# RupertLuo/Valley

Measured on AMD Instinct MI355X. Metric: frames/sec ViT-L/14 encode + prefill tokens/sec (13B), higher is better.
Workload: dtype bf16

## Files before the change

valley_amd/csrc/attention.hip:

```cpp
#include <cstdlib>
#include "common.hpp"
#include "../../include/valley_hip.h"

namespace {

constexpr float LOG2E = 1.4426950408889634f;
constexpr float NEG_BIG = -1.0e30f;

#ifndef VLY_DECODE_MERGE_FENCE
#define VLY_DECODE_MERGE_FENCE 0
#endif
#ifndef VLY_VIT_PRIO
#define VLY_VIT_PRIO 0
#endif
#ifndef VLY_VIT_STAGGER
#define VLY_VIT_STAGGER 0
#endif
#ifndef VLY_VIT_TIMING
#define VLY_VIT_TIMING 0
#endif
#ifndef VLY_VIT_STAGE2
#define VLY_VIT_STAGE2 1
#endif
#ifndef VLY_VIT_ROT
#define VLY_VIT_ROT 0
#endif
#ifndef VLY_VIT_FOLD
#define VLY_VIT_FOLD 0
#endif
#ifndef VLY_VIT_STORE_LINES
#define VLY_VIT_STORE_LINES 0
#endif
#ifndef VLY_FAST_EXP2
#define VLY_FAST_EXP2 1
#endif
VLY_DEVICE float sm_exp2(float x) {
#if VLY_FAST_EXP2
    return __builtin_amdgcn_exp2f(x);
#else
    return exp2f(x);
#endif
}

VLY_DEVICE uint32_t sel16(const u32x4& a, const u32x4& b, int dd) {
    const uint32_t w = dd < 8 ? a[dd >> 1] : b[(dd - 8) >> 1];
    return (dd & 1) ? (w >> 16) : (w & 0xffffu);
}

VLY_DEVICE int opaque_i32(int v) {
    asm volatile("" : "+v"(v));
    return v;
}

VLY_DEVICE void store_tile_rows(uint16_t* row_ptr, const f32x4 (&o)[4], float inv, int g) {
    uint32_t y[2][4];
#pragma unroll
    for (int w = 0; w < 2; ++w) {
        uint32_t d[4];
#pragma unroll
        for (int dt = 0; dt < 4; ++dt) d[dt] = pack_h2(o[dt][2 * w] * inv, o[dt][2 * w + 1] * inv);
        const auto p01 = __builtin_amdgcn_permlane16_swap(d[0], d[1], false, false);
        const auto p23 = __builtin_amdgcn_permlane16_swap(d[2], d[3], false, false);
        const auto q0 = __builtin_amdgcn_permlane32_swap(p01[0], p23[0], false, false);
        const auto q1 = __builtin_amdgcn_permlane32_swap(p01[1], p23[1], false, false);
        y[w][0] = q0[0]; y[w][1] = q1[0]; y[w][2] = q0[1]; y[w][3] = q1[1];
    }
    u32x4* dst = (u32x4*)(row_ptr + 16 * g);
    dst[0] = u32x4{y[0][0], y[1][0], y[0][1], y[1][1]};
    dst[1] = u32x4{y[0][2], y[1][2], y[0][3], y[1][3]};
}

template <typename OP>
VLY_DEVICE float rows4_reduce(float v, OP op) {
    {
        const uint32_t x = __float_as_uint(v);
        const auto r = __builtin_amdgcn_permlane16_swap(x, x, false, false);
        v = op(__uint_as_float(r[0]), __uint_as_float(r[1]));
    }
    {
        const uint32_t x = __float_as_uint(v);
        const auto r = __builtin_amdgcn_permlane32_swap(x, x, false, false);
        v = op(__uint_as_float(r[0]), __uint_as_float(r[1]));
    }
    return v;
}
VLY_DEVICE float rows4_max(float v) { return rows4_reduce(v, [](float a, float b) { return fmaxf(a, b); }); }
VLY_DEVICE float rows4_sum(float v) { return rows4_reduce(v, [](float a, float b) { return a + b; }); }

constexpr int VN = 257;
constexpr int VNT = 17;
constexpr int VNC = 9;
constexpr int VLD = 3072;
constexpr int VT_STRIDE = 296;
constexpr int VK_BYTES = VNT * 16 * 128;

constexpr int VNW = 8;

#if VLY_VIT_TIMING
constexpr int VTS_WG = 4096, VTS_N = 24;
__device__ unsigned long long vit_ts[VTS_WG * VNW * VTS_N];
#define VLY_VSTAMP()                                                                                     \
    do {                                                                                                  \
        if (ts_row && lane == 0 && tsn < VTS_N) ts_row[tsn] = __builtin_readcyclecounter();                \
        ++tsn;                                                                                            \
    } while (0)
#else
#define VLY_VSTAMP() do {} while (0)
#endif

__global__ void __launch_bounds__(VNW * 64, 4) vit_attn_kernel(const uint16_t* __restrict__ qkv, uint16_t* __restrict__ out) {
    __shared__ __attribute__((aligned(16))) char smem[VK_BYTES + 64 * VT_STRIDE * 2];
    char* sK = smem;
    uint16_t* sVt = (uint16_t*)(smem + VK_BYTES);

    const int tid = threadIdx.x, lane = tid & 63, wave = tid >> 6;
    const int l15 = lane & 15, g = lane >> 4;
    [[maybe_unused]] const int hi16 = opaque_i32(16);
    const int h = blockIdx.x & 15;
#if VLY_VIT_TIMING
    int tsn = 0;
    unsigned long long* ts_row = blockIdx.x < VTS_WG ? vit_ts + ((size_t)blockIdx.x * VNW + wave) * VTS_N : nullptr;
    VLY_VSTAMP();
    if (ts_row && lane == 0) {
        unsigned hw, xcc;
        asm volatile("s_getreg_b32 %0, hwreg(HW_REG_HW_ID)" : "=s"(hw));
        asm volatile("s_getreg_b32 %0, hwreg(HW_REG_XCC_ID)" : "=s"(xcc));
        ts_row[tsn] = (unsigned long long)hw | ((unsigned long long)xcc << 32);
    }
    ++tsn;
#endif
    const int f = blockIdx.x >> 4;
    const uint16_t* base = qkv + (size_t)f * VN * VLD + h * 64;

#if VLY_VIT_STAGE2
    const int dq = wave & 3;
    u32x4 kr[5];
#pragma unroll
    for (int i = 0; i < 5; ++i) {
        const int sl = tid + i * VNW * 64, row = min(sl >> 3, VN - 1), c = sl & 7;
        kr[i] = *(const u32x4*)(base + (size_t)row * VLD + 1024 + c * 8);
    }
    u32x4 vr[2][4];
#pragma unroll
    for (int ps = 0; ps < 2; ++ps) {
        const int pg = ps == 0 ? (wave >> 2) : 2, kv0 = 2 * (pg * 64 + lane), kv1 = kv0 + 1;
        if (ps == 0 || wave < 4) {
            const uint16_t* r0 = base + (size_t)min(kv0, VN - 1) * VLD + 2048 + dq * 16;
            const uint16_t* r1 = base + (size_t)min(kv1, VN - 1) * VLD + 2048 + dq * 16;
            vr[ps][0] = *(const u32x4*)r0;
            vr[ps][1] = *(const u32x4*)(r0 + 8);
            vr[ps][2] = *(const u32x4*)r1;
            vr[ps][3] = *(const u32x4*)(r1 + 8);
        }
// ... 234 lines not shown
#if VLY_VIT_TIMING
    if (ts_row && lane == 0 && tsn < VTS_N) ts_row[VTS_N - 1] = (unsigned long long)tsn;
#endif
}
#undef VLY_VSTAMP

typedef __attribute__((ext_vector_type(4))) short s16x4;
#include "attention_vit_persist.inc"
#include "attention_vit_pp.inc"

#ifndef VLY_LNW
#define VLY_LNW 8
#endif
constexpr int LNW = VLY_LNW;

VLY_DEVICE bf16x8 vt_frag256(const char* lo_addr) {
    typedef __attribute__((address_space(3))) s16x4 lds_s16x4;
    const s16x4 lo = __builtin_amdgcn_ds_read_tr16_b64_v4i16((lds_s16x4*)(lo_addr));
    const s16x4 hi = __builtin_amdgcn_ds_read_tr16_b64_v4i16((lds_s16x4*)(lo_addr + 16 * 256));
    return bf16x8{lo[0], lo[1], lo[2], lo[3], hi[0], hi[1], hi[2], hi[3]};
}

constexpr int L2_TILE = 64 * 256;
constexpr int L2_BUF = 2 * L2_TILE;

__global__ void __launch_bounds__(LNW * 64, 4) llama_attn2_kernel(const uint16_t* __restrict__ qkv, const uint16_t* __restrict__ kc,
                                                                 const uint16_t* __restrict__ vc, const uint8_t* __restrict__ key_valid,
                                                                 uint16_t* __restrict__ out, int S, int heads, int past,
                                                                 const int32_t* __restrict__ past_dev, int kv_stride, int ctx_max) {
    static_assert(LNW == 8, "16 + 16 pieces on 8 waves");
    __shared__ __attribute__((aligned(16))) char smem[2 * L2_BUF];
    const int tid = threadIdx.x, lane = tid & 63;
    const int wave = __builtin_amdgcn_readfirstlane(tid >> 6);
    const int l15 = lane & 15, g = lane >> 4;
    const int h = blockIdx.x, b = blockIdx.y, qb = (int)gridDim.z - 1 - (int)blockIdx.z;
    const int Hq = heads * 128;
    if (past_dev) past = min(*past_dev, ctx_max - S);
    const int kv_len = past + S;

    const int q = qb * (LNW * 16) + wave * 16 + l15;
    const int qc = min(q, S - 1);
    const int qpos = past + q;
    const int q_last = min(qb * (LNW * 16) + LNW * 16 - 1, S - 1);
    const int wave_qpos_max = past + min(qb * (LNW * 16) + wave * 16 + 15, S - 1);
    const int kv_end = min(past + q_last + 1, kv_len);
    const int ntiles = (kv_end + 63) >> 6;

    const size_t head_off = ((size_t)b * heads + h) * (size_t)ctx_max * 128;
    const __amdgpu_buffer_rsrc_t rsK = vly_rsrc(kc + head_off), rsV = vly_rsrc(vc + head_off);
    const __amdgpu_buffer_rsrc_t rsM = vly_rsrc(key_valid ? key_valid + (size_t)b * kv_stride : key_valid);
    const uint32_t lds0 = (uint32_t)(uintptr_t)(__attribute__((address_space(3))) char*)smem;
    const uint32_t hb = 0u;
    uint32_t okraw = 1u;
    bool okin = false;
    auto stage = [&](int kt, int buf) {
        const int kv0 = kt * 64;
#pragma unroll
        for (int pp = 0; pp < 2; ++pp) {
            const int pc = 2 * wave + pp, row = 4 * pc + (lane >> 4), cp = lane & 15;
            const uint32_t rb = hb + (uint32_t)min(kv0 + row, kv_len - 1) * 256u;
            const uint32_t voK = rb + (uint32_t)((cp ^ (row & 15)) << 4);
            const uint32_t voV = rb + (uint32_t)((cp ^ ((row & 7) << 1)) << 4);
            const uint32_t dst = __builtin_amdgcn_readfirstlane(lds0 + (uint32_t)buf * L2_BUF + (uint32_t)pc * 1024u);
            asm volatile("s_mov_b32 m0, %0" ::"s"(dst) : "memory");
            asm volatile("s_nop 0" ::: "memory");
            asm volatile("buffer_load_dwordx4 %0, %1, 0 offen lds" ::"v"(voK), "s"(rsK) : "memory");
            asm volatile("s_mov_b32 m0, %0" ::"s"(dst + (uint32_t)L2_TILE) : "memory");
            asm volatile("s_nop 0" ::: "memory");
            asm volatile("buffer_load_dwordx4 %0, %1, 0 offen lds" ::"v"(voV), "s"(rsV) : "memory");
        }
        const int kvl = kv0 + lane;
        okin = kvl < kv_len;
        if (key_valid) okraw = (uint32_t)__builtin_amdgcn_raw_buffer_load_b8(rsM, (uint32_t)min(kvl, kv_len - 1), 0, 0);
    };
    const int vr = 4 * g + (l15 >> 2);
    const int vbase0 = L2_TILE + vr * 256 + (l15 & 1) * 8 + (((l15 & 3) >> 1) << 4), vx0 = (vr & 7) << 5;

    if (ntiles > 0) stage(0, 0);
    const uint16_t* qp = qkv + ((size_t)b * S + qc) * 3 * Hq + h * 128;
    bf16x8 qf[4];
#pragma unroll
    for (int kk = 0; kk < 4; ++kk) qf[kk] = *(const bf16x8*)(qp + kk * 32 + g * 8);

    const float sc = 0.08838834764831845f * LOG2E;
    float m = NEG_BIG, l = 0.f;
    f32x4 o[8];
#pragma unroll
    for (int dt = 0; dt < 8; ++dt) o[dt] = f32x4{0.f, 0.f, 0.f, 0.f};

    for (int kt = 0; kt < ntiles; ++kt) {
        const int kv0 = kt * 64, buf = kt & 1;
        const char* sK = smem + buf * L2_BUF;
        __builtin_amdgcn_s_waitcnt(0x0f70);
        __syncthreads();
        const unsigned long long vmask = __ballot(okin && (okraw & 0xffu) != 0u);
        if (kt + 1 < ntiles) stage(kt + 1, buf ^ 1);
        if (kv0 > wave_qpos_max) continue;
        const int vbase = opaque_i32(vbase0), vx = opaque_i32(vx0);

        f32x4 s[4];
#pragma unroll
        for (int t = 0; t < 4; ++t) {
            f32x4 acc = {0.f, 0.f, 0.f, 0.f};
#pragma unroll
            for (int kk = 0; kk < 4; ++kk) {
                const bf16x8 kf = *(const bf16x8*)(sK + (t * 16 + l15) * 256 + (((kk * 4 + g) ^ l15) << 4));
                acc = mfma16(kf, qf[kk], acc);
            }
#pragma unroll
            for (int r = 0; r < 4; ++r) {
                const int kl = t * 16 + 4 * g + r;
                const bool vis = ((vmask >> kl) & 1ull) && (kv0 + kl <= qpos);
                s[t][r] = vis ? acc[r] * sc : NEG_BIG;
            }
        }
        float rm = NEG_BIG;
#pragma unroll
        for (int t = 0; t < 4; ++t)
#pragma unroll
            for (int r = 0; r < 4; ++r) rm = fmaxf(rm, s[t][r]);
        rm = rows4_max(rm);
        const float mn = fmaxf(m, rm);
        const float alpha = sm_exp2(m - mn);
        m = mn;
        float ps = 0.f;
#pragma unroll
        for (int t = 0; t < 4; ++t)
#pragma unroll
            for (int r = 0; r < 4; ++r) {
                const float p = sm_exp2(s[t][r] - mn);
                s[t][r] = p;
                ps += p;
            }
        l = l * alpha + ps;
#pragma unroll
        for (int dt = 0; dt < 8; ++dt) o[dt] *= alpha;
#pragma unroll
        for (int c = 0; c < 2; ++c) {
            u32x4 pk;
            pk[0] = pack_h2(s[2 * c][0], s[2 * c][1]);
            pk[1] = pack_h2(s[2 * c][2], s[2 * c][3]);
            pk[2] = pack_h2(s[2 * c + 1][0], s[2 * c + 1][1]);
            pk[3] = pack_h2(s[2 * c + 1][2], s[2 * c + 1][3]);
            const bf16x8 pf = __builtin_bit_cast(bf16x8, pk);
#pragma unroll
            for (int dt = 0; dt < 8; ++dt)
                o[dt] = mfma16(vt_frag256(sK + vbase + ((dt << 5) ^ vx) + c * 8192), pf, o[dt]);
        }
    }
    l = rows4_sum(l);
    if (q < S) {
        const float inv = 1.f / l;
        uint16_t* op = out + ((size_t)b * S + q) * Hq + h * 128 + 4 * g;
#pragma unroll
        for (int dt = 0; dt < 8; ++dt) {
            u32x2 pk;
            pk[0] = pack_h2(o[dt][0] * inv, o[dt][1] * inv);
            pk[1] = pack_h2(o[dt][2] * inv, o[dt][3] * inv);
            *(u32x2*)(op + dt * 16) = pk;
        }
    }
}

constexpr int DEC_MAX_CTX = 8192;

__global__ void __launch_bounds__(256) decode_attn_kernel(const uint16_t* __restrict__ qkv, const uint16_t* __restrict__ kc,
                                                          const uint16_t* __restrict__ vc, const uint8_t* __restrict__ key_valid,
                                                          uint16_t* __restrict__ out, int heads, int past,
                                                          const int32_t* __restrict__ past_dev, int kv_stride, int ctx_max) {
    __shared__ float sc[DEC_MAX_CTX];
    __shared__ __attribute__((aligned(16))) float qs[128];
    __shared__ float red[8];
    __shared__ __attribute__((aligned(16))) float acc_s[16][128];
    const int tid = threadIdx.x, lane = tid & 63, wave = tid >> 6;
    const int h = blockIdx.x, b = blockIdx.y;
    const int Hq = heads * 128;
    if (past_dev) past = min(*past_dev, ctx_max - 1);
    const int kv_len = past + 1;
    const uint16_t* qp = qkv + (size_t)b * 3 * Hq + h * 128;
    if (tid < 128) qs[tid] = h2f(qp[tid]) * (0.08838834764831845f * LOG2E);
    __syncthreads();
    const uint16_t* kbase = kc + ((size_t)b * heads + h) * ctx_max * 128;
    const uint16_t* vbase = vc + ((size_t)b * heads + h) * ctx_max * 128;
    const uint8_t* kvld = key_valid ? key_valid + (size_t)b * kv_stride : nullptr;

    float m = NEG_BIG;
    for (int j = tid; j < kv_len; j += 256) {
        float s = NEG_BIG;
        if (!kvld || kvld[j]) {
            const u32x4* kr = (const u32x4*)(kbase + (size_t)j * 128);
            float a = 0.f;
#pragma unroll
            for (int c = 0; c < 16; ++c) {
                const u32x4 kk = kr[c];
                const f32x4 q0 = *(const f32x4*)(qs + 8 * c), q1 = *(const f32x4*)(qs + 8 * c + 4);
                a = fmaf(h_lo(kk[0]), q0[0], a); a = fmaf(h_hi(kk[0]), q0[1], a);
                a = fmaf(h_lo(kk[1]), q0[2], a); a = fmaf(h_hi(kk[1]), q0[3], a);
                a = fmaf(h_lo(kk[2]), q1[0], a); a = fmaf(h_hi(kk[2]), q1[1], a);
                a = fmaf(h_lo(kk[3]), q1[2], a); a = fmaf(h_hi(kk[3]), q1[3], a);
            }
            s = a;
        }
        sc[j] = s;
        m = fmaxf(m, s);
    }
    m = wave_max(m);
    if (lane == 0) red[wave] = m;
    __syncthreads();
    m = fmaxf(fmaxf(red[0], red[1]), fmaxf(red[2], red[3]));
    float l = 0.f;
    for (int j = tid; j < kv_len; j += 256) {
        const float p = sm_exp2(sc[j] - m);
        sc[j] = p;
        l += p;
    }
    l = wave_sum(l);
    if (lane == 0) red[4 + wave] = l;
    __syncthreads();
    l = red[4] + red[5] + red[6] + red[7];

    const int kg = tid >> 4, dc = tid & 15;
    float o[8];
#pragma unroll
    for (int i = 0; i < 8; ++i) o[i] = 0.f;
    for (int j0 = kg; j0 < kv_len; j0 += 64) {
        u32x4 vv[4];
        float pp[4];
#pragma unroll
        for (int u = 0; u < 4; ++u) {
            const int j = j0 + 16 * u;
            const bool in = j < kv_len;
            pp[u] = in ? sc[j] : 0.f;
            vv[u] = *(const u32x4*)(vbase + (size_t)(in ? j : kg) * 128 + 8 * dc);
        }
#pragma unroll
        for (int u = 0; u < 4; ++u) {
            const float p = pp[u];
            o[0] = fmaf(p, h_lo(vv[u][0]), o[0]); o[1] = fmaf(p, h_hi(vv[u][0]), o[1]);
            o[2] = fmaf(p, h_lo(vv[u][1]), o[2]); o[3] = fmaf(p, h_hi(vv[u][1]), o[3]);
            o[4] = fmaf(p, h_lo(vv[u][2]), o[4]); o[5] = fmaf(p, h_hi(vv[u][2]), o[5]);
            o[6] = fmaf(p, h_lo(vv[u][3]), o[6]); o[7] = fmaf(p, h_hi(vv[u][3]), o[7]);
        }
    }
#pragma unroll
    for (int i = 0; i < 8; ++i) acc_s[kg][8 * dc + i] = o[i];
    __syncthreads();
    if (tid < 128) {
        float t = 0.f;
#pragma unroll
        for (int k2 = 0; k2 < 16; ++k2) t += acc_s[k2][tid];
        out[(size_t)b * Hq + h * 128 + tid] = f2h(t / l);
    }
}

__global__ void __launch_bounds__(512) decode_fused_kernel(const uint16_t* __restrict__ qkv, uint16_t* __restrict__ kc,
                                                           uint16_t* __restrict__ vc, const float* __restrict__ cos_t,
                                                           const float* __restrict__ sin_t, const uint8_t* __restrict__ key_valid,
                                                           uint16_t* __restrict__ out, int heads, int past,
                                                           const int32_t* __restrict__ past_dev, int kv_stride, int ctx_max,
                                                           int past_row_stride) {
    __shared__ float sc[512];
    __shared__ __attribute__((aligned(16))) float qs[128];
    __shared__ __attribute__((aligned(16))) float knew[128];
    __shared__ __attribute__((aligned(16))) float vnew[128];
    __shared__ float red[16];
    __shared__ __attribute__((aligned(16))) float acc_s[32][128];
    const int tid = threadIdx.x, lane = tid & 63, wave = tid >> 6;
    const int h = blockIdx.x, b = blockIdx.y;
    const int Hq = heads * 128;
    if (past_dev) past = min(past_dev[(size_t)b * past_row_stride], ctx_max - 1);
    const int pos = past, kv_len = past + 1;
    const uint16_t* qp = qkv + (size_t)b * 3 * Hq + h * 128;
    uint16_t* kbase = kc + ((size_t)b * heads + h) * ctx_max * 128;
    uint16_t* vbase = vc + ((size_t)b * heads + h) * ctx_max * 128;
    const uint8_t* kvld = key_valid ? key_valid + (size_t)b * kv_stride : nullptr;

    if (tid < 64) {
        const float cs = cos_t[(size_t)pos * 64 + tid], sn = sin_t[(size_t)pos * 64 + tid];
        const float q0 = h2f(qp[tid]), q1 = h2f(qp[tid + 64]);
        const float k0 = h2f(qp[Hq + tid]), k1 = h2f(qp[Hq + tid + 64]);
        const float scale = 0.08838834764831845f * LOG2E;
        qs[tid] = h2f(f2h(rope_rot(q0, q1, cs, sn, -1.f))) * scale;
        qs[tid + 64] = h2f(f2h(rope_rot(q1, q0, cs, sn, 1.f))) * scale;
        const uint16_t r0 = f2h(rope_rot(k0, k1, cs, sn, -1.f)), r1 = f2h(rope_rot(k1, k0, cs, sn, 1.f));
        knew[tid] = h2f(r0);
        knew[tid + 64] = h2f(r1);
        kbase[(size_t)pos * 128 + tid] = r0;
        kbase[(size_t)pos * 128 + tid + 64] = r1;
    } else if (tid < 192) {
        const int d = tid - 64;
        const uint16_t v = qp[2 * Hq + d];
        vnew[d] = h2f(v);
        vbase[(size_t)pos * 128 + d] = v;
    }
    __syncthreads();

    const int kg = tid >> 4, dc = tid & 15;
    float o[8];
#pragma unroll
    for (int i = 0; i < 8; ++i) o[i] = 0.f;
    float m_run = NEG_BIG, l_run = 0.f;

    for (int c0 = 0; c0 < kv_len; c0 += 512) {
        u32x4 vv[16];
#pragma unroll
        for (int u = 0; u < 16; ++u) {
// ... 244 lines not shown
        __syncthreads();
        lc = red[4] + red[5] + red[6] + red[7];
        l_run = vly_mul_add(l_run, alpha, lc);
        m_run = m_new;
#pragma unroll
        for (int i = 0; i < 8; ++i) o[i] *= alpha;
#pragma unroll
        for (int u = 0; u < 16; ++u) {
            const int jl = kg + 16 * u;
            const float pj = sc[jl];
            if (owner && c0 + jl == pos) {
#pragma unroll
                for (int i = 0; i < 8; ++i) o[i] = fmaf(pj, vnew[8 * dc + i], o[i]);
            } else {
                o[0] = fmaf(pj, h_lo(vv[u][0]), o[0]); o[1] = fmaf(pj, h_hi(vv[u][0]), o[1]);
                o[2] = fmaf(pj, h_lo(vv[u][1]), o[2]); o[3] = fmaf(pj, h_hi(vv[u][1]), o[3]);
                o[4] = fmaf(pj, h_lo(vv[u][2]), o[4]); o[5] = fmaf(pj, h_hi(vv[u][2]), o[5]);
                o[6] = fmaf(pj, h_lo(vv[u][3]), o[6]); o[7] = fmaf(pj, h_hi(vv[u][3]), o[7]);
            }
        }
        __syncthreads();
    }
#pragma unroll
    for (int i = 0; i < 8; ++i) acc_s[kg][8 * dc + i] = o[i];
    __syncthreads();
    if (tid < 128) {
        float t = 0.f;
#pragma unroll
        for (int k2 = 0; k2 < 16; ++k2) t += acc_s[k2][tid];
        split_publish(part + 4 + tid, t, merged != nullptr);
    } else if (tid < 132) {
        split_publish(part + tid - 128, tid == 128 ? m_run : tid == 129 ? l_run : 0.f, merged != nullptr);
    }
    if (merged) split_merge_if_last(partials, merged, arrivals, heads, h, b, sc);
}


template <typename T> VLY_DEVICE float probs_ld(const T* p);
template <> VLY_DEVICE float probs_ld<uint16_t>(const uint16_t* p) { return h2f(*p); }
template <> VLY_DEVICE float probs_ld<float>(const float* p) { return *p; }

template <typename T>
__global__ void __launch_bounds__(256) attn_probs_kernel(const T* __restrict__ qkv, const T* __restrict__ kc,
                                                         const uint8_t* __restrict__ key_valid, float* __restrict__ out, int S,
                                                         int heads, int past, int kv_stride, int ctx_max) {
    extern __shared__ float pr_sc[];
    __shared__ float qs[128];
    __shared__ float red[8];
    const int tid = threadIdx.x, lane = tid & 63, wave = tid >> 6;
    const int i = blockIdx.x, h = blockIdx.y, b = blockIdx.z;
    const int kv_len = past + S, vis = past + i + 1, Hq = heads * 128;
    const T* q = qkv + ((size_t)b * S + i) * 3 * Hq + h * 128;
    const T* kb = kc + ((size_t)b * heads + h) * ctx_max * 128;
    const uint8_t* kvld = key_valid ? key_valid + (size_t)b * kv_stride : nullptr;
    if (tid < 128) qs[tid] = probs_ld(q + tid) * (0.08838834764831845f * LOG2E);
    __syncthreads();
    float m = NEG_BIG;
    for (int j = tid; j < kv_len; j += 256) {
        float s = NEG_BIG;
        if (j < vis && (!kvld || kvld[j])) {
            const T* kr = kb + (size_t)j * 128;
            float a = 0.f;
#pragma unroll 8
            for (int d = 0; d < 128; ++d) a = fmaf(probs_ld(kr + d), qs[d], a);
            s = a;
        }
        pr_sc[j] = s;
        m = fmaxf(m, s);
    }
    m = wave_max(m);
    if (lane == 0) red[wave] = m;
    __syncthreads();
    m = fmaxf(fmaxf(red[0], red[1]), fmaxf(red[2], red[3]));
    float l = 0.f;
    for (int j = tid; j < kv_len; j += 256) {
        const float s = pr_sc[j];
        const float p = s > 0.5f * NEG_BIG ? sm_exp2(s - m) : 0.f;
        pr_sc[j] = p;
        l += p;
    }
    l = wave_sum(l);
    if (lane == 0) red[4 + wave] = l;
    __syncthreads();
    l = red[4] + red[5] + red[6] + red[7];
    const float inv = l > 0.f ? 1.f / l : 0.f;
    float* o = out + (((size_t)b * heads + h) * S + i) * kv_len;
    for (int j = tid; j < kv_len; j += 256) o[j] = pr_sc[j] * inv;
}

#ifndef VLY_EXPERIMENTAL
#define VLY_EXPERIMENTAL 0
#endif
#if VLY_EXPERIMENTAL
#include "attention_ab.inc"
#endif

}

#if VLY_VIT_TIMING
extern "C" int vlydbg_vit_timing_read(unsigned long long* host) { return (int)hipMemcpyFromSymbol(host, HIP_SYMBOL(vit_ts), sizeof(unsigned long long) * VTS_WG * VNW * VTS_N); }
#endif

#ifndef VLY_VIT_PERSIST_MIN
#define VLY_VIT_PERSIST_MIN 1
#endif
#ifndef VLY_VIT_PP
#define VLY_VIT_PP 0
#endif
constexpr int VIT_PERSIST_MIN_FRAMES = VLY_VIT_PERSIST_MIN;
extern "C" int vly_vit_attention(const void* qkv, void* out, int F, void* stream) {
    if (F <= 0 || ((uintptr_t)qkv & 15) || ((uintptr_t)out & 15)) { vly_set_error("vly_vit_attention: bad args F=%d (qkv and out 16-byte aligned)", F); return -22; }
    const char* sel = getenv("VLY_VIT_ATTN");
    const int ver = sel ? atoi(sel) : 0;
    if (ver == 4 || ver == 5 || (ver != 1 && F >= VIT_PERSIST_MIN_FRAMES)) {
        static const int cus = [] {
            int dev = 0, n = 0;
            (void)hipGetDevice(&dev);
            (void)hipDeviceGetAttribute(&n, hipDeviceAttributeMultiprocessorCount, dev);
            return n > 0 ? n : 256;
        }();
        const int nheads = F * 16;
        if ((size_t)F * VN * VLD * 2 >= ((size_t)1 << 32)) { vly_set_error("vly_vit_attention: F=%d exceeds the 4 GB buffer descriptor", F); return -22; }
        if (ver == 5 || VLY_VIT_PP) {
            hipLaunchKernelGGL(vit_attn_pp_kernel, dim3(nheads < 2 * cus ? nheads : 2 * cus), dim3(PPW * 64), 0, (hipStream_t)stream,
                               (const uint16_t*)qkv, (uint16_t*)out, nheads);
            return vly_check_launch("vly_vit_attention");
        }
        hipLaunchKernelGGL(vit_attn_persist_kernel, dim3(nheads < cus ? nheads : cus), dim3(VPW * 64), 0, (hipStream_t)stream,
                           (const uint16_t*)qkv, (uint16_t*)out, nheads);
        return vly_check_launch("vly_vit_attention");
    }
    hipLaunchKernelGGL(vit_attn_kernel, dim3(F * 16), dim3(VNW * 64), 0, (hipStream_t)stream, (const uint16_t*)qkv, (uint16_t*)out);
    return vly_check_launch("vly_vit_attention");
}

extern "C" int vly_llama_attention(const void* qkv, const void* kcache, const void* vcache, const uint8_t* key_valid,
                                   int key_valid_stride, void* out, int B, int S, int heads, int past_len,
                                   const int32_t* past_len_dev, int ctx_max, void* stream) {
    if (B <= 0 || S <= 0 || heads <= 0 || past_len < 0 || past_len + S > ctx_max || B > 65535 || heads > 65535 ||
        ((uintptr_t)qkv & 15) || ((uintptr_t)kcache & 15) || ((uintptr_t)vcache & 15) || ((uintptr_t)out & 7)) {
        vly_set_error("vly_llama_attention: bad args B=%d S=%d heads=%d past=%d ctx_max=%d", B, S, heads, past_len, ctx_max);
        return -22;
    }
    if (key_valid && key_valid_stride < past_len + S) {
        vly_set_error("vly_llama_attention: key_valid_stride %d < kv_len %d", key_valid_stride, past_len + S);
        return -22;
    }
    if (S == 1 && ctx_max <= DEC_MAX_CTX) {
        hipLaunchKernelGGL(decode_attn_kernel, dim3(heads, B), dim3(256), 0, (hipStream_t)stream, (const uint16_t*)qkv,
                           (const uint16_t*)kcache, (const uint16_t*)vcache, key_valid, (uint16_t*)out, heads, past_len,
                           past_len_dev, key_valid_stride, ctx_max);
        return vly_check_launch("vly_llama_attention(decode)");
    }
#if VLY_EXPERIMENTAL
    static const int ver = getenv("VLY_LLAMA_ATTN") ? atoi(getenv("VLY_LLAMA_ATTN")) : 2;
#else
    constexpr int ver = 2;
#endif
    if ((size_t)ctx_max * 256 >= ((size_t)1 << 32)) {
        vly_set_error("vly_llama_attention: ctx_max %d exceeds the 4 GB a (batch, head) cache row may span", ctx_max);
        return -22;
    }
    if (ver == 2) {
        hipLaunchKernelGGL(llama_attn2_kernel, dim3(heads, B, (S + 16 * LNW - 1) / (16 * LNW)), dim3(LNW * 64), 0, (hipStream_t)stream,
                           (const uint16_t*)qkv, (const uint16_t*)kcache, (const uint16_t*)vcache, key_valid, (uint16_t*)out,
                           S, heads, past_len, past_len_dev, key_valid_stride, ctx_max);
        return vly_check_launch("vly_llama_attention");
    }
#if VLY_EXPERIMENTAL
    hipLaunchKernelGGL(llama_attn_kernel, dim3(heads, B, (S + 16 * LNW - 1) / (16 * LNW)), dim3(LNW * 64), 0, (hipStream_t)stream,
                       (const uint16_t*)qkv, (const uint16_t*)kcache, (const uint16_t*)vcache, key_valid, (uint16_t*)out,
                       S, heads, past_len, past_len_dev, key_valid_stride, ctx_max);
    return vly_check_launch("vly_llama_attention");
#else
    return -22;
#endif
}

extern "C" int vly_decode_attention(const void* qkv, void* kcache, void* vcache, const float* cos_table, const float* sin_table,
                                    const uint8_t* key_valid, int key_valid_stride, void* out, int B, int heads, int past_len,
                                    const int32_t* past_len_dev, int ctx_max, void* stream) {
    if (B <= 0 || heads <= 0 || past_len < 0 || past_len + 1 > ctx_max || B > 65535 || heads > 65535 ||
        ((uintptr_t)qkv & 15) || ((uintptr_t)kcache & 15) || ((uintptr_t)vcache & 15) || ((uintptr_t)out & 7) || !cos_table || !sin_table) {
        vly_set_error("vly_decode_attention: bad args B=%d heads=%d past=%d ctx_max=%d", B, heads, past_len, ctx_max);
        return -22;
    }
    if (key_valid && key_valid_stride < past_len + 1) {
        vly_set_error("vly_decode_attention: key_valid_stride %d < kv_len %d", key_valid_stride, past_len + 1);
        return -22;
    }
    hipLaunchKernelGGL(decode_fused_kernel, dim3(heads, B), dim3(512), 0, (hipStream_t)stream, (const uint16_t*)qkv,
                       (uint16_t*)kcache, (uint16_t*)vcache, cos_table, sin_table, key_valid, (uint16_t*)out, heads, past_len,
                       past_len_dev, key_valid_stride, ctx_max, 0);
    return vly_check_launch("vly_decode_attention");
}

extern "C" int vly_decode_attention_rows(const void* qkv, void* kcache, void* vcache, const float* cos_table, const float* sin_table,
                                         const uint8_t* key_valid, int key_valid_stride, void* out, int B, int heads,
                                         const int32_t* past_len_rows, int ctx_max, void* stream) {
    if (B <= 0 || heads <= 0 || !past_len_rows || B > 65535 || heads > 65535 || ((uintptr_t)qkv & 15) || ((uintptr_t)kcache & 15) ||
        ((uintptr_t)vcache & 15) || ((uintptr_t)out & 7) || !cos_table || !sin_table || (key_valid && key_valid_stride < ctx_max)) {
        vly_set_error("vly_decode_attention_rows: bad args B=%d heads=%d ctx_max=%d key_valid_stride=%d", B, heads, ctx_max, key_valid_stride);
        return -22;
    }
    hipLaunchKernelGGL(decode_fused_kernel, dim3(heads, B), dim3(512), 0, (hipStream_t)stream, (const uint16_t*)qkv,
                       (uint16_t*)kcache, (uint16_t*)vcache, cos_table, sin_table, key_valid, (uint16_t*)out, heads, 0,
                       past_len_rows, key_valid_stride, ctx_max, 1);
    return vly_check_launch("vly_decode_attention_rows");
}

static int decode_split_launch(const char* name, const void* qkv, void* kcache, void* vcache, const float* cos_table,
                               const float* sin_table, const uint8_t* key_valid, int key_valid_stride, float* partials, int B,
                               int heads, int past_len, const int32_t* past_len_dev, int past_len_dev_stride, int ctx_max,
                               void* merged, unsigned* arrivals, void* stream);

#if VLY_EXPERIMENTAL
extern "C" int vly_decode_attention_split(const void* qkv, void* kcache, void* vcache, const float* cos_table, const float* sin_table,
                                          const uint8_t* key_valid, int key_valid_stride, float* partials, int B, int heads,
                                          int past_len, const int32_t* past_len_dev, int past_len_dev_stride, int ctx_max,
                                          void* stream) {
    return decode_split_launch("vly_decode_attention_split", qkv, kcache, vcache, cos_table, sin_table, key_valid, key_valid_stride,
                               partials, B, heads, past_len, past_len_dev, past_len_dev_stride, ctx_max, nullptr, nullptr, stream);
}
#endif

extern "C" int vly_decode_attention_merged(const void* qkv, void* kcache, void* vcache, const float* cos_table, const float* sin_table,
                                           const uint8_t* key_valid, int key_valid_stride, float* partials, void* out,
                                           uint32_t* arrivals, int B, int heads, int past_len, const int32_t* past_len_dev,
                                           int past_len_dev_stride, int ctx_max, void* stream) {
    if (!out || ((uintptr_t)out & 7) || !arrivals || ((uintptr_t)arrivals & 3)) {
        vly_set_error("vly_decode_attention_merged: out (8-byte aligned) and arrivals (B * heads zeroed uint32) are required");
        return -22;
    }
    return decode_split_launch("vly_decode_attention_merged", qkv, kcache, vcache, cos_table, sin_table, key_valid, key_valid_stride,
                               partials, B, heads, past_len, past_len_dev, past_len_dev_stride, ctx_max, out, arrivals, stream);
}

static int decode_split_launch(const char* name, const void* qkv, void* kcache, void* vcache, const float* cos_table,
                               const float* sin_table, const uint8_t* key_valid, int key_valid_stride, float* partials, int B,
                               int heads, int past_len, const int32_t* past_len_dev, int past_len_dev_stride, int ctx_max,
                               void* merged, unsigned* arrivals, void* stream) {
    if (B <= 0 || heads <= 0 || past_len < 0 || past_len + 1 > ctx_max || B > 65535 || heads > 65535 || ((uintptr_t)qkv & 15) ||
        ((uintptr_t)kcache & 15) || ((uintptr_t)vcache & 15) || !partials || ((uintptr_t)partials & 15) || !cos_table || !sin_table ||
        past_len_dev_stride < 0 || past_len_dev_stride > 1 || (past_len_dev_stride == 1 && !past_len_dev)) {
        vly_set_error("%s: bad args B=%d heads=%d past=%d ctx_max=%d", name, B, heads, past_len, ctx_max);
        return -22;
    }
    if (key_valid && key_valid_stride < (past_len_dev ? ctx_max : past_len + 1)) {
        vly_set_error("%s: key_valid_stride %d too short", name, key_valid_stride);
        return -22;
    }
    static const bool spread = getenv("VLY_DECODE_SPLIT_SPREAD") && atoi(getenv("VLY_DECODE_SPLIT_SPREAD")) != 0 && VLY_DECODE_SPLITS != 1;
    const dim3 grid = spread && B != VLY_DECODE_SPLITS ? dim3(VLY_DECODE_SPLITS, heads, B) : dim3(heads, B, VLY_DECODE_SPLITS);
    hipLaunchKernelGGL(decode_split_kernel, grid, dim3(256), 0, (hipStream_t)stream, (const uint16_t*)qkv,
                       (uint16_t*)kcache, (uint16_t*)vcache, cos_table, sin_table, key_valid, partials, heads, past_len, past_len_dev,
                       key_valid_stride, ctx_max, past_len_dev_stride, (uint16_t*)merged, arrivals);
    return vly_check_launch(name);
}

extern "C" int vly_llama_attention_probs(const void* qkv, const void* kcache, const uint8_t* key_valid, int key_valid_stride,
                                         float* out, int B, int S, int heads, int past_len, int ctx_max, int inputs_f32,
                                         void* stream) {
    const int kv_len = past_len + S;
    if (B <= 0 || S <= 0 || heads <= 0 || past_len < 0 || kv_len > ctx_max || kv_len > 16000 || B > 65535 || heads > 65535 || !qkv ||
        !kcache || !out) {
        vly_set_error("vly_llama_attention_probs: bad args B=%d S=%d heads=%d past=%d ctx_max=%d (kv_len <= 16000)", B, S, heads,
                      past_len, ctx_max);
        return -22;
    }
    if (key_valid && key_valid_stride < kv_len) {
        vly_set_error("vly_llama_attention_probs: key_valid_stride %d < kv_len %d", key_valid_stride, kv_len);
        return -22;
    }
    const dim3 grid(S, heads, B), block(256);
    const size_t lds = (size_t)kv_len * 4;
    if (inputs_f32)
        hipLaunchKernelGGL(attn_probs_kernel<float>, grid, block, lds, (hipStream_t)stream, (const float*)qkv, (const float*)kcache,
                           key_valid, out, S, heads, past_len, key_valid_stride, ctx_max);
    else
        hipLaunchKernelGGL(attn_probs_kernel<uint16_t>, grid, block, lds, (hipStream_t)stream, (const uint16_t*)qkv,
                           (const uint16_t*)kcache, key_valid, out, S, heads, past_len, key_valid_stride, ctx_max);
    return vly_check_launch("vly_llama_attention_probs");
}
```

Measured before the change: 1749.

## Add causal-aware prefill attention kernel with per-wave tile skipping and specialization

Adds a new llama_attn3 prefill attention kernel and makes it the default. Each wave skips KV tiles fully past its causal horizon and bounds the KV loop by the block's last query. Fully visible tiles take an unmasked fast path, and diagonal tiles are compiled for 1-4 live 16-column sub-tiles to avoid wasted MFMAs. Query blocks are launched in reverse order so the heaviest blocks start first. The default now reads an environment variable on every call, and the kernel is more complex with more specialized code paths.

Result: no change. 1752, median of 4 (+0.2%).

```diff
diff --git a/valley_amd/csrc/attention.hip b/valley_amd/csrc/attention.hip
--- a/valley_amd/csrc/attention.hip
+++ b/valley_amd/csrc/attention.hip
@@ -1,4 +1,5 @@
 #include <cstdlib>
+#include <type_traits>
 #include "common.hpp"
 #include "../../include/valley_hip.h"
 
@@ -539,6 +540,187 @@
     if (q < S) {
         const float inv = 1.f / l;
         uint16_t* op = out + ((size_t)b * S + q) * Hq + h * 128 + 4 * g;
+#pragma unroll
+        for (int dt = 0; dt < 8; ++dt) {
+            u32x2 pk;
+            pk[0] = pack_h2(o[dt][0] * inv, o[dt][1] * inv);
+            pk[1] = pack_h2(o[dt][2] * inv, o[dt][3] * inv);
+            *(u32x2*)(op + dt * 16) = pk;
+        }
+    }
+}
+
+__global__ void __launch_bounds__(LNW * 64, 4) llama_attn3_kernel(const uint16_t* __restrict__ qkv, const uint16_t* __restrict__ kc,
+                                                                 const uint16_t* __restrict__ vc, const uint8_t* __restrict__ key_valid,
+                                                                 uint16_t* __restrict__ out, int S, int heads, int past,
+                                                                 const int32_t* __restrict__ past_dev, int kv_stride, int ctx_max) {
+    static_assert(LNW == 8, "16 + 16 pieces on 8 waves");
+    __shared__ __attribute__((aligned(16))) char smem[2 * L2_BUF];
+    const int tid = threadIdx.x, lane = tid & 63;
+    const int wave = __builtin_amdgcn_readfirstlane(tid >> 6);
+    const int l15 = lane & 15, g = lane >> 4;
+    const int h = blockIdx.x, b = blockIdx.y, qb = (int)gridDim.z - 1 - (int)blockIdx.z;
+    const int Hq = heads * 128;
+    if (past_dev) past = min(*past_dev, ctx_max - S);
+    const int kv_len = past + S;
+
+    const int w0 = qb * (LNW * 16) + wave * 16;
+    const bool live = w0 < S;
+    const int q = w0 + l15;
+    const int qc = min(q, S - 1);
+    const int qpos = past + q;
+    const int q_last = min(qb * (LNW * 16) + LNW * 16 - 1, S - 1);
+    const int wave_qpos_min = past + w0;
+    const int wave_qpos_max = live ? past + min(w0 + 15, S - 1) : -1;
+    const int kv_end = min(past + q_last + 1, kv_len);
+    const int ntiles = (kv_end + 63) >> 6;
+
+    const size_t head_off = ((size_t)b * heads + h) * (size_t)ctx_max * 128;
+    const __amdgpu_buffer_rsrc_t rsK = vly_rsrc(kc + head_off), rsV = vly_rsrc(vc + head_off);
+    const __amdgpu_buffer_rsrc_t rsM = vly_rsrc(key_valid ? key_valid + (size_t)b * kv_stride : key_valid);
+    const uint32_t lds0 = (uint32_t)(uintptr_t)(__attribute__((address_space(3))) char*)smem;
+    uint32_t okraw = 1u;
+    bool okin = false;
+    auto stage = [&](int kt, int buf) {
+        const int kv0 = kt * 64;
+        const int sl = opaque_i32(lane), sl15 = sl & 15;
+        const int row0 = 8 * wave + (sl >> 4), swK0 = (sl15 ^ (row0 & 15)) << 4, swV0 = (sl15 ^ ((row0 & 7) << 1)) << 4;
+#pragma unroll
+        for (int pp = 0; pp < 2; ++pp) {
+            const int pc = 2 * wave + pp, row = row0 + 4 * pp;
+            const uint32_t rb = (uint32_t)min(kv0 + row, kv_len - 1) * 256u;
+            const uint32_t voK = rb + (uint32_t)(swK0 ^ (pp << 6));
+            const uint32_t voV = rb + (uint32_t)(swV0 ^ (pp << 7));
+            const uint32_t dst = __builtin_amdgcn_readfirstlane(lds0 + (uint32_t)buf * L2_BUF + (uint32_t)pc * 1024u);
+            asm volatile("s_mov_b32 m0, %0" ::"s"(dst) : "memory");
+            asm volatile("s_nop 0" ::: "memory");
+            asm volatile("buffer_load_dwordx4 %0, %1, 0 offen lds" ::"v"(voK), "s"(rsK) : "memory");
+            asm volatile("s_mov_b32 m0, %0" ::"s"(dst + (uint32_t)L2_TILE) : "memory");
+            asm volatile("s_nop 0" ::: "memory");
+            asm volatile("buffer_load_dwordx4 %0, %1, 0 offen lds" ::"v"(voV), "s"(rsV) : "memory");
+        }
+        const int kvl = kv0 + sl;
+        okin = kvl < kv_len;
+        if (key_valid && live) okraw = (uint32_t)__builtin_amdgcn_raw_buffer_load_b8(rsM, (uint32_t)min(kvl, kv_len - 1), 0, 0);
+    };
+
+    if (ntiles > 0) stage(0, 0);
+    bf16x8 qf[4] = {};
+    if (live) {
+        const uint16_t* qp = qkv + ((size_t)b * S + qc) * 3 * Hq + h * 128;
+#pragma unroll
+        for (int kk = 0; kk < 4; ++kk) qf[kk] = *(const bf16x8*)(qp + kk * 32 + g * 8);
+    }
+
+    const float sc = 0.08838834764831845f * LOG2E;
+    float m = NEG_BIG, l = 0.f;
+    f32x4 o[8];
+#pragma unroll
+    for (int dt = 0; dt < 8; ++dt) o[dt] = f32x4{0.f, 0.f, 0.f, 0.f};
+
+    for (int kt = 0; kt < ntiles; ++kt) {
+        const int kv0 = kt * 64, buf = kt & 1;
+        const char* sK = smem + buf * L2_BUF;
+        __builtin_amdgcn_s_waitcnt(0x0f70);
+        __syncthreads();
+        const unsigned long long vmask = __ballot(okin && (okraw & 0xffu) != 0u);
+        if (kt + 1 < ntiles) stage(kt + 1, buf ^ 1);
+        if (kv0 > wave_qpos_max) continue;
+        const int tl = opaque_i32(lane), tl15 = tl & 15, tg = tl >> 4, vr = 4 * tg + (tl15 >> 2);
+        const int krow = tl15 * 256 + ((tg ^ tl15) << 4);
+        const int vbase = L2_TILE + vr * 256 + (tl15 & 1) * 8 + (((tl15 & 3) >> 1) << 4), vx = (vr & 7) << 5;
+
+        const auto tile = [&](auto nl_c, auto masked_c) {
+            constexpr int NL = decltype(nl_c)::value;
+            constexpr bool MASKED = decltype(masked_c)::value;
+            f32x4 s[4];
+            uint32_t vw[2] = {0u, 0u};
+            if (MASKED) {
+                const int dd = qpos - kv0 - 4 * tg;
+                const unsigned long long cm = dd >= 63 ? ~0ull : dd < 0 ? 0ull : (2ull << dd) - 1ull;
+                const unsigned long long vm = (vmask >> (4 * tg)) & cm;
+                vw[0] = (uint32_t)vm;
+                vw[1] = (uint32_t)(vm >> 32);
+            }
+#pragma unroll
+            for (int t = 0; t < NL; ++t) {
+                f32x4 acc = {0.f, 0.f, 0.f, 0.f};
+#pragma unroll
+                for (int kk = 0; kk < 4; ++kk) {
+                    const bf16x8 kf = *(const bf16x8*)(sK + t * 4096 + (krow ^ (kk << 6)));
+                    acc = mfma16(kf, qf[kk], acc);
+                }
+#pragma unroll
+                for (int r = 0; r < 4; ++r) {
+                    if (MASKED) {
+                        const bool vis = (vw[t >> 1] >> ((t & 1) * 16 + r)) & 1u;
+                        s[t][r] = vis ? acc[r] * sc : NEG_BIG;
+                    } else {
+                        float v = acc[r] * sc;
+                        asm("" : "+v"(v));
+                        s[t][r] = v;
+                    }
+                }
+            }
+            float rm = NEG_BIG;
+#pragma unroll
+            for (int t = 0; t < NL; ++t)
+#pragma unroll
+                for (int r = 0; r < 4; ++r) rm = fmaxf(rm, s[t][r]);
+            rm = rows4_max(rm);
+            const float mn = fmaxf(m, rm);
+            const float alpha = sm_exp2(m - mn);
+            m = mn;
+            float ps = 0.f;
+#pragma unroll
+            for (int t = 0; t < NL; ++t)
+#pragma unroll
+                for (int r = 0; r < 4; ++r) {
+                    const float p = sm_exp2(s[t][r] - mn);
+                    s[t][r] = p;
+                    ps += p;
+                }
+            uint32_t pkd = 0u;
+            if (NL < 4) {
+                const float pd = sm_exp2(NEG_BIG - mn);
+                if (__any(pd != 0.f)) {
+#pragma unroll
+                    for (int i = 0; i < 4 * (4 - NL); ++i) ps += pd;
+                }
+                pkd = pack_h2(pd, pd);
+            }
+            l = l * alpha + ps;
+#pragma unroll
+            for (int dt = 0; dt < 8; ++dt) o[dt] *= alpha;
+#pragma unroll
+            for (int c = 0; c < 2; ++c) {
+                u32x4 pk = {pkd, pkd, pkd, pkd};
+                if (2 * c < NL) {
+                    pk[0] = pack_h2(s[2 * c][0], s[2 * c][1]);
+                    pk[1] = pack_h2(s[2 * c][2], s[2 * c][3]);
+                }
+                if (2 * c + 1 < NL) {
+                    pk[2] = pack_h2(s[2 * c + 1][0], s[2 * c + 1][1]);
+                    pk[3] = pack_h2(s[2 * c + 1][2], s[2 * c + 1][3]);
+                }
+                const bf16x8 pf = __builtin_bit_cast(bf16x8, pk);
+#pragma unroll
+                for (int dt = 0; dt < 8; ++dt)
+                    o[dt] = mfma16(vt_frag256(sK + vbase + ((dt << 5) ^ vx) + c * 8192), pf, o[dt]);
+            }
+        };
+        const int nl = ((wave_qpos_max - kv0) >> 4) + 1;
+        if (kv0 + 63 <= wave_qpos_min && vmask == ~0ull) tile(std::integral_constant<int, 4>{}, std::false_type{});
+        else if (nl >= 4) tile(std::integral_constant<int, 4>{}, std::true_type{});
+        else if (nl == 3) tile(std::integral_constant<int, 3>{}, std::true_type{});
+        else if (nl == 2) tile(std::integral_constant<int, 2>{}, std::true_type{});
+        else tile(std::integral_constant<int, 1>{}, std::true_type{});
+    }
+    l = rows4_sum(l);
+    const int el = opaque_i32(lane), eq = w0 + (el & 15);
+    if (eq < S) {
+        const float inv = 1.f / l;
+        uint16_t* op = out + ((size_t)b * S + eq) * Hq + h * 128 + 4 * (el >> 4);
 #pragma unroll
         for (int dt = 0; dt < 8; ++dt) {
             u32x2 pk;
@@ -1089,14 +1271,22 @@
                            past_len_dev, key_valid_stride, ctx_max);
         return vly_check_launch("vly_llama_attention(decode)");
     }
+    const char* sel = getenv("VLY_LLAMA_ATTN");
+    const int asked = sel ? atoi(sel) : 3;
 #if VLY_EXPERIMENTAL
-    static const int ver = getenv("VLY_LLAMA_ATTN") ? atoi(getenv("VLY_LLAMA_ATTN")) : 2;
+    const int ver = asked == 1 || asked == 2 ? asked : 3;
 #else
-    constexpr int ver = 2;
+    const int ver = asked == 2 ? 2 : 3;
 #endif
     if ((size_t)ctx_max * 256 >= ((size_t)1 << 32)) {
         vly_set_error("vly_llama_attention: ctx_max %d exceeds the 4 GB a (batch, head) cache row may span", ctx_max);
         return -22;
+    }
+    if (ver == 3) {
+        hipLaunchKernelGGL(llama_attn3_kernel, dim3(heads, B, (S + 16 * LNW - 1) / (16 * LNW)), dim3(LNW * 64), 0, (hipStream_t)stream,
+                           (const uint16_t*)qkv, (const uint16_t*)kcache, (const uint16_t*)vcache, key_valid, (uint16_t*)out,
+                           S, heads, past_len, past_len_dev, key_valid_stride, ctx_max);
+        return vly_check_launch("vly_llama_attention");
     }
     if (ver == 2) {
         hipLaunchKernelGGL(llama_attn2_kernel, dim3(heads, B, (S + 16 * LNW - 1) / (16 * LNW)), dim3(LNW * 64), 0, (hipStream_t)stream,
```
